# 0xPolygonZero/plonky

Hardware: AMD Instinct MI355X
Metric: MSM Mpairs/sec + NTT Melems/sec, 2^20 Tweedledee, 1/2/4/8 GPU (higher is better)
Workload: dtype u32; 1 GPU; 2^20 TweedledeeBase forward NTT + 2^20-pair tweedledee MSM per GPU per step; log_n=20, curve=tweedledee

## Files before the change

### plonky_amd/csrc/msm_geom.h

```cpp
#pragma once
#include <stddef.h>
#include <stdint.h>
#include <stdio.h>

#include "../../include/plonky_hip.h"
#include "glv_params.cuh"

namespace plk {

constexpr int ACC_THREADS = 128;

constexpr int MSM_MAX_PLANE_PARTS = 16;
constexpr int MSM_TF_MAX_WINDOW = 16;
constexpr int MSM_MAX_WINDOW = 21;
constexpr uint32_t CODE_INVALID = 0xFFFFFFFFu;
constexpr int ORD_THREADS = 256;
constexpr int ORD_TILE = 4096;
constexpr int ORD_MAX_BINS = 1024;
constexpr int ORD_MAX_FINE = 11;
constexpr int ORD_BIN_THREADS = 512;
constexpr uint32_t ORD_SEG = 8192;
constexpr int ORD_SEG_EPT = (int)(ORD_SEG / ORD_BIN_THREADS);
static_assert(3 * (4u << ORD_MAX_FINE) + 4 * ORD_BIN_THREADS + 6 * ORD_SEG <= 160 * 1024, "k_ord_bin_scatter's LDS tile must fit a gfx950 CU");
constexpr uint32_t ORD2_BIN_CAP = 32768;
constexpr int PLANE_THREADS = 512;
constexpr int FINAL_FUSE_WINDOWS = 4;
constexpr int FINAL_THREADS = 512;
constexpr int COMBINE_THREADS = 512;
constexpr uint32_t HEAD_NONE = 0xFFFFFFFFu;
constexpr uint32_t HEAVY_HEADS = 32;
constexpr uint32_t HEAVY_CHUNK = 2048;

struct OrdCfg {
    int c;
    int windows;
    uint32_t window_buckets;
    int fine_bits;
    int nbins;
    uint32_t spt;
    uint32_t sub;
    uint32_t nt1;
    int raw_signed;
    uint32_t entries_cap;
    uint32_t ent_stride;
    uint32_t ent_first;
    int perm;
    uint32_t bin_lo, bin_hi;
};

struct TailGeom {
    uint32_t buckets, heavy_cap, tail_wbuckets;
    int lpb_log;
    int two_level;
    int L, H, g_log, lpl_log;
    int table_free, windows;
    int tail_windows;
    int plane_blocks;
    int planes;
    int tail_shift;
    int transposed;
    int many_heads;
};

constexpr int META_BIN_TOTAL = 0;
constexpr int META_BIN_BASE = META_BIN_TOTAL + ORD_MAX_BINS;
constexpr int META_SEG_BASE = META_BIN_BASE + ORD_MAX_BINS + 1;
constexpr int META_DONE = META_SEG_BASE + ORD_MAX_BINS + 1;
constexpr int META_FINAL_DONE = META_DONE + 1;
constexpr int META_DYN_CHUNK = META_DONE + 2;
constexpr int META_LIVE_COUNT = META_DONE + 3;
constexpr int META_WORDS = META_DONE + 8;

enum MsmPart {
    PART_TMP,
    PART_SORTED,
    PART_CNT1,
    PART_CNT2,
    PART_META,
    PART_OFF,
    PART_P_START,
    PART_P_HEAD,
    PART_HEAD_LIVE,
    PART_BUCKET,
    PART_HEAVY,
    PART_HEAVY_PART,
    PART_LINE_PART,
    PART_PLANE_PART,
    PART_WIN_PTS,
    MSM_WORK_PARTS
};

inline size_t head_lanes_padded(size_t max_lanes) { return (max_lanes + ACC_THREADS + 15) & ~(size_t)15; }

struct MsmKnob {
    bool set = false;
    int v = 0;
};
struct MsmKnobs {
    MsmKnob window;
    MsmKnob window_2p14;
    MsmKnob window_tf;
    MsmKnob glog;
    int slice = 0;
    int comb = -1;
    bool no_glv = false;
    bool order_v1 = false;
};

struct MsmGeom {
    int c = 0;
    int windows = 0;
    uint32_t buckets = 0;
    uint32_t wbuckets = 0;
    bool table_free = false;
    bool glv = false;
    size_t n_eff = 0;
    OrdCfg ord{};
    TailGeom tail{};
    uint32_t chunk = 24;
    size_t max_lanes = 0;
    uint32_t heavy_cap = 0;
    size_t part_bytes[MSM_WORK_PARTS] = {};
    char error[192] = {};
};

constexpr int msm_scalar_bits(int curve) {
    return curve == PLK_CURVE_BLS12_377 ? 253 : (curve >= PLK_CURVE_TWEEDLEDEE && curve <= PLK_CURVE_VESTA) ? 255 : -1;
}

inline int ilog2_ceil(uint64_t v) {
    int b = 0;
    while (((uint64_t)1 << b) < v) ++b;
    return b;
}

inline int choose_window(size_t n, int curve, const MsmKnobs& knobs) {
    int lg = 0;
    while (((size_t)1 << (lg + 1)) <= n) ++lg;
    const int bits = msm_scalar_bits(curve) + 1;
    auto digits = [&](int c) { return (bits + c - 1) / c; };
    auto top_bits = [&](int c) { return bits - (digits(c) - 1) * c; };
    int c;
    if (lg >= 14) {
        double best = 0;
        c = 0;
        for (int t = 10; t <= MSM_MAX_WINDOW - 1; ++t) {
            const double acc = 10.0 * (double)n * digits(t);
            const double cost = acc + 28.0 * (double)((size_t)1 << (t - 1)) + (2 * top_bits(t) < t ? 0.1 * acc : 0.0);
            if (c == 0 || cost < best) {
                best = cost;
                c = t;
            }
        }
// ... 176 lines not shown
```

### plonky_amd/csrc/msm_order.hip

```cpp
#include "msm_dev.cuh"
#include "glv.cuh"
#include <cstdlib>

namespace plk {


struct OrdRaw {
    uint4 lo, hi;
};
PLK_DI OrdRaw ord_load_scalar(const uint4* __restrict__ scalars, size_t i, bool live) {
    OrdRaw r;
    r.lo = r.hi = make_uint4(0u, 0u, 0u, 0u);
    if (live) {
        r.lo = scalars[i * 2];
        r.hi = scalars[i * 2 + 1];
    }
    return r;
}
template <class SP> PLK_DI void ord_park_loaded(const OrdRaw& r, uint32_t* s_lim, int tid, bool raw_signed) {
    static_assert(SP::NL == 8, "scalar fields are 256-bit");
    Fe<SP> s;
    s.v[0] = r.lo.x; s.v[1] = r.lo.y; s.v[2] = r.lo.z; s.v[3] = r.lo.w;
    s.v[4] = r.hi.x; s.v[5] = r.hi.y; s.v[6] = r.hi.z; s.v[7] = r.hi.w;
    if (!raw_signed) s = fe_to_canonical<SP>(s);
#pragma unroll
    for (int k = 0; k < 8; ++k) s_lim[k * ORD_THREADS + tid] = s.v[k];
}
template <class SP> PLK_DI void ord_park_scalar(const uint4* __restrict__ scalars, size_t i, uint32_t* s_lim, int tid, bool raw_signed) {
    ord_park_loaded<SP>(ord_load_scalar(scalars, i, true), s_lim, tid, raw_signed);
}
PLK_DI uint32_t ord_digit(const uint32_t* s_lim, int tid, int j, const OrdCfg& cfg, uint32_t& carry) {
    const int c = cfg.c;
    const uint32_t mask = (1u << c) - 1u, half = 1u << (c - 1);
    const int bp = j * c, li = bp >> 5, sh = bp & 31;
    uint64_t two = li < 8 ? s_lim[li * ORD_THREADS + tid] : 0u;
    if (li + 1 < 8) two |= (uint64_t)s_lim[(li + 1) * ORD_THREADS + tid] << 32;
    const uint32_t v = ((uint32_t)(two >> sh) & mask) + carry;
    const uint32_t neg = v > half ? 1u : 0u;
    const uint32_t mag = neg ? (1u << c) - v : v;
    carry = neg;
    if (mag == 0) return CODE_INVALID;
    const uint32_t flip = cfg.raw_signed ? s_lim[7 * ORD_THREADS + tid] >> 31 : 0u;
    return ((mag - 1u + (uint32_t)j * cfg.window_buckets) << 1) | (neg ^ flip);
}

PLK_DI bool ord_bin_kept(uint32_t bin, const OrdCfg& cfg) { return bin - cfg.bin_lo < cfg.bin_hi - cfg.bin_lo; }

PLK_DI uint32_t block_excl_prefix(uint32_t v, uint32_t* s_tmp, uint32_t* total = nullptr) {
    const int t = threadIdx.x, lane = t & 63, wave = t >> 6, nw = blockDim.x >> 6;
    uint32_t inc = v;
#pragma unroll
    for (int d = 1; d < 64; d <<= 1) {
        const uint32_t u = __shfl_up(inc, d);
        if (lane >= d) inc += u;
    }
    if (lane == 63) s_tmp[wave] = inc;
    __syncthreads();
    uint32_t base = 0, all = 0;
    for (int w = 0; w < nw; ++w) {
        const uint32_t x = s_tmp[w];
        if (w < wave) base += x;
        all += x;
    }
    if (total) *total = all;
    __syncthreads();
    return base + inc - v;
}
PLK_DI void block_excl_scan4(uint32_t* s_data, int count, uint32_t* s_tmp) {
    const int t = threadIdx.x;
    uint32_t v[4], sum = 0;
#pragma unroll
    for (int k = 0; k < 4; ++k) {
        const int idx = t * 4 + k;
        v[k] = idx < count ? s_data[idx] : 0u;
        sum += v[k];
    }
    uint32_t run = block_excl_prefix(sum, s_tmp);
#pragma unroll
    for (int k = 0; k < 4; ++k) {
        const int idx = t * 4 + k;
        if (idx < count) s_data[idx] = run;
        run += v[k];
    }
    __syncthreads();
// ... 220 lines not shown
    __syncthreads();
#pragma unroll
    for (int k = 0; k < ORD_SEG_EPT; ++k)
        if (lo + tid + k * ORD_BIN_THREADS < hi) atomicAdd(&s_hist[(code[k] >> 1) & fmask], 1u);
    __syncthreads();
    for (int k = tid; k < nf; k += ORD_BIN_THREADS) cnt2[((size_t)blockIdx.x << fine_bits) + k] = s_hist[k];
}
__global__ void __launch_bounds__(ORD_BIN_THREADS) k_ord_bin_scatter(const uint2* __restrict__ tmp, const uint32_t* __restrict__ bin_base,
                                                                     const uint32_t* __restrict__ seg_base, int fine_bits, int nbins, uint32_t buckets,
                                                                     const uint32_t* __restrict__ cnt2, uint32_t* __restrict__ off,
                                                                     uint32_t* __restrict__ sorted, uint32_t entries_cap) {
    __shared__ uint32_t s_glob[1 << ORD_MAX_FINE], s_loc[1 << ORD_MAX_FINE], s_cur[1 << ORD_MAX_FINE];
    __shared__ uint32_t s_tmp[ORD_BIN_THREADS];
    __shared__ uint32_t s_out[ORD_SEG];
    __shared__ uint16_t s_fine[ORD_SEG];
    const int tid = threadIdx.x;
    uint32_t bin, seg, lo, hi;
    if (!ord_segment(seg_base, bin_base, nbins, blockIdx.x, bin, seg, lo, hi)) {
        const uint32_t extra = blockIdx.x - seg_base[nbins];
        if (extra < (uint32_t)nbins && bin_base[extra + 1] == bin_base[extra]) {
            const int nf = 1 << fine_bits;
            for (int k = tid; k < nf; k += ORD_BIN_THREADS) off[((size_t)extra << fine_bits) + k] = bin_base[extra];
        }
        if (extra == 0 && tid == 0) off[buckets] = bin_base[nbins];
        return;
    }
    const int nf = 1 << fine_bits;
    const uint32_t fmask = (uint32_t)nf - 1u;
    uint2 ent[ORD_SEG_EPT];
#pragma unroll
    for (int k = 0; k < ORD_SEG_EPT; ++k) {
        const uint32_t p = lo + tid + k * ORD_BIN_THREADS;
        ent[k] = tmp[p < hi ? p : lo];
    }
    const uint32_t s0 = seg_base[bin], s1 = seg_base[bin + 1];
    for (int k = tid; k < nf; k += ORD_BIN_THREADS) {
        uint32_t tot = 0, before = 0, own = 0;
        for (uint32_t sg = s0; sg < s1; ++sg) {
            const uint32_t v = cnt2[((size_t)sg << fine_bits) + k];
            if (sg - s0 < seg) before += v;
            if (sg - s0 == seg) own = v;
            tot += v;
        }
        s_glob[k] = tot;
        s_cur[k] = before;
        s_loc[k] = own;
    }
    __syncthreads();
    block_excl_scan4(s_glob, nf, s_tmp);
    block_excl_scan4(s_loc, nf, s_tmp);
    const uint32_t bb = bin_base[bin];
    for (int k = tid; k < nf; k += ORD_BIN_THREADS) {
        const uint32_t o = bb + s_glob[k];
        if (seg == 0) off[((size_t)bin << fine_bits) + k] = o;
        s_glob[k] = o + s_cur[k];
        s_cur[k] = s_loc[k];
    }
    __syncthreads();
#pragma unroll
    for (int k = 0; k < ORD_SEG_EPT; ++k) {
        if (lo + tid + k * ORD_BIN_THREADS >= hi) continue;
        const uint2 e = ent[k];
        const uint32_t f = (e.x >> 1) & fmask;
        const uint32_t idx = atomicAdd(&s_cur[f], 1u);
        if (PLK_CHK(idx < ORD_SEG, CHK_SEG_STAGE)) {
            s_out[idx] = (e.y << 1) | (e.x & 1u);
            s_fine[idx] = (uint16_t)f;
        }
    }
    __syncthreads();
    const uint32_t count = hi - lo;
    for (uint32_t i = tid; i < count; i += ORD_BIN_THREADS) {
        const uint32_t f = s_fine[i];
        const uint32_t at = s_glob[f] + (i - s_loc[f]);
        if (PLK_CHK(at < entries_cap, CHK_SORTED_INDEX)) sorted[at] = s_out[i];
    }
}


constexpr int ORD2_TS = 1024;
constexpr int ORD2_THREADS = 512;
constexpr int ORD2_SPT = ORD2_TS / ORD2_THREADS;
constexpr int ORD2_MAX_WINDOWS = 16;
constexpr uint32_t ORD2_MAX_TILES = 8192;
PLK_DI uint32_t ord2_record(uint32_t sign, uint32_t fine, int j, uint32_t loc) { return sign | (fine << 1) | ((uint32_t)j << 12) | (loc << 16); }
PLK_DI uint32_t ord_digit_at(const uint32_t* s_lim, int stride, int slot, int j, const OrdCfg& cfg, uint32_t& carry) {
    const int c = cfg.c;
    const uint32_t mask = (1u << c) - 1u, half = 1u << (c - 1);
    const int bp = j * c, li = bp >> 5, sh = bp & 31;
    uint64_t two = li < 8 ? s_lim[li * stride + slot] : 0u;
    if (li + 1 < 8) two |= (uint64_t)s_lim[(li + 1) * stride + slot] << 32;
    const uint32_t v = ((uint32_t)(two >> sh) & mask) + carry;
    const uint32_t neg = v > half ? 1u : 0u;
    const uint32_t mag = neg ? (1u << c) - v : v;
    carry = neg;
    if (mag == 0) return CODE_INVALID;
    const uint32_t flip = cfg.raw_signed ? s_lim[7 * stride + slot] >> 31 : 0u;
    return ((mag - 1u + (uint32_t)j * cfg.window_buckets) << 1) | (neg ^ flip);
}
struct OrdWalk {
    uint32_t w[8];
    uint32_t carry, flip;
};
template <class SP> PLK_DI void ord_walk_start(OrdWalk& s, const Fe<SP>& canon, const OrdCfg& cfg) {
#pragma unroll
    for (int k = 0; k < 8; ++k) s.w[k] = canon.v[k];
    s.carry = 0;
    s.flip = cfg.raw_signed ? canon.v[7] >> 31 : 0u;
}
PLK_DI uint32_t ord_walk_next(OrdWalk& s, int j, const OrdCfg& cfg) {
    const int c = cfg.c;
    const uint32_t mask = (1u << c) - 1u, half = 1u << (c - 1);
    const uint32_t v = (s.w[0] & mask) + s.carry;
#pragma unroll
    for (int k = 0; k < 7; ++k) s.w[k] = (s.w[k] >> c) | (s.w[k + 1] << (32 - c));
    s.w[7] >>= c;
    const uint32_t neg = v > half ? 1u : 0u;
    const uint32_t mag = neg ? (1u << c) - v : v;
    s.carry = neg;
    if (mag == 0) return CODE_INVALID;
    return ((mag - 1u + (uint32_t)j * cfg.window_buckets) << 1) | (neg ^ s.flip);
}
template <class C>
__global__ void __launch_bounds__(ORD2_THREADS) k_ord_tiles(const uint4* __restrict__ scalars, size_t n, OrdCfg cfg, uint32_t* __restrict__ cnt1,
                                                            uint32_t* __restrict__ bin_total, uint32_t* __restrict__ tmp) {
    using SP = typename C::SP;
    static_assert(SP::NL == 8, "scalar fields are 256-bit");
    __shared__ uint32_t s_cnt[ORD_MAX_BINS], s_base[ORD_MAX_BINS];
    __shared__ uint32_t s_tmp[ORD2_THREADS];
    __shared__ uint32_t s_total;
    extern __shared__ __attribute__((aligned(16))) uint32_t s_ent[];
    const int tid = threadIdx.x;
    const uint32_t tile = blockIdx.x;
    const uint32_t cap = (uint32_t)ORD2_TS * (uint32_t)cfg.windows;
    static_assert(ORD2_SPT == 2, "two scalars per thread, held in named registers (an indexed array of them is promoted to LDS by the compiler: 32 KiB)");
    const size_t i0 = (size_t)tile * ORD2_TS + tid, i1 = i0 + ORD2_THREADS;
    const bool live0 = i0 < n, live1 = i1 < n;
    const OrdRaw raw0 = ord_load_scalar(scalars, i0, live0), raw1 = ord_load_scalar(scalars, i1, live1);
    for (int k = tid; k < cfg.nbins; k += ORD2_THREADS) s_cnt[k] = 0;
    auto canonical = [&](const OrdRaw& r) {
        Fe<SP> sc;
        sc.v[0] = r.lo.x; sc.v[1] = r.lo.y; sc.v[2] = r.lo.z; sc.v[3] = r.lo.w;
        sc.v[4] = r.hi.x; sc.v[5] = r.hi.y; sc.v[6] = r.hi.z; sc.v[7] = r.hi.w;
        if (!cfg.raw_signed) sc = fe_to_canonical<SP>(sc);
        return sc;
    };
    const Fe<SP> canon0 = canonical(raw0), canon1 = canonical(raw1);
    __syncthreads();
    const int cbits = cfg.c - 1 - cfg.fine_bits;
    const uint32_t bmask = (1u << cbits) - 1u;
    uint32_t code0[ORD2_MAX_WINDOWS], code1[ORD2_MAX_WINDOWS];
    {
        OrdWalk w0, w1;
        ord_walk_start<SP>(w0, canon0, cfg);
        ord_walk_start<SP>(w1, canon1, cfg);
#pragma unroll
        for (int j = 0; j < ORD2_MAX_WINDOWS; ++j) {
            code0[j] = (j < cfg.windows && live0) ? ord_walk_next(w0, j, cfg) : CODE_INVALID;
            code1[j] = (j < cfg.windows && live1) ? ord_walk_next(w1, j, cfg) : CODE_INVALID;
            if (code0[j] != CODE_INVALID && !ord_bin_kept((code0[j] >> 1) & bmask, cfg)) code0[j] = CODE_INVALID;
            if (code1[j] != CODE_INVALID && !ord_bin_kept((code1[j] >> 1) & bmask, cfg)) code1[j] = CODE_INVALID;
        }
    }
#pragma unroll
    for (int j = 0; j < ORD2_MAX_WINDOWS; ++j) {
        if (code0[j] != CODE_INVALID) atomicAdd(&s_cnt[(code0[j] >> 1) & bmask], 1u);
        if (code1[j] != CODE_INVALID) atomicAdd(&s_cnt[(code1[j] >> 1) & bmask], 1u);
    }
    __syncthreads();
    for (int k = tid; k < cfg.nbins; k += ORD2_THREADS) s_base[k] = s_cnt[k];
    __syncthreads();
    block_excl_scan4(s_base, cfg.nbins, s_tmp);
    if (tid == 0) s_total = s_base[cfg.nbins - 1] + s_cnt[cfg.nbins - 1];
    for (int k = tid; k < cfg.nbins; k += ORD2_THREADS) {
        const uint32_t cn = s_cnt[k];
        cnt1[(size_t)k * cfg.nt1 + tile] = (s_base[k] << 16) | cn;
        if (cn) atomicAdd(&bin_total[k], cn);
    }
    __syncthreads();
#pragma unroll
    for (int j = 0; j < ORD2_MAX_WINDOWS; ++j) {
        if (code0[j] != CODE_INVALID) {
            const uint32_t slot = atomicAdd(&s_base[(code0[j] >> 1) & bmask], 1u);
            if (PLK_CHK(slot < cap, CHK_TILE_STAGE)) s_ent[slot] = ord2_record(code0[j] & 1u, code0[j] >> (cbits + 1), j, (uint32_t)tid);
        }
        if (code1[j] != CODE_INVALID) {
            const uint32_t slot = atomicAdd(&s_base[(code1[j] >> 1) & bmask], 1u);
            if (PLK_CHK(slot < cap, CHK_TILE_STAGE)) s_ent[slot] = ord2_record(code1[j] & 1u, code1[j] >> (cbits + 1), j, (uint32_t)(ORD2_THREADS + tid));
        }
    }
    __syncthreads();
    const uint32_t total = s_total;
    uint32_t* __restrict__ region = tmp + (size_t)tile * cap;
    for (uint32_t i = tid; i < total; i += ORD2_THREADS)
        if (PLK_CHK((size_t)tile * cap + i < (size_t)cfg.nt1 * cap, CHK_TMP_INDEX)) region[i] = s_ent[i];
}

__global__ void __launch_bounds__(256) k_ord_scan_bins(uint32_t* __restrict__ bin_total, int nbins, uint32_t* __restrict__ bin_base,
                                                       uint32_t* __restrict__ seg_base, uint32_t* __restrict__ dyn_chunk, uint32_t chunk_cfg,
                                                       uint32_t lanes_cfg, uint32_t hot) {
    __shared__ uint32_t s_sum[256];
    __shared__ uint32_t s_bins[ORD_MAX_BINS], s_tot[ORD_MAX_BINS];
    for (int k = threadIdx.x; k < nbins; k += 256) {
        s_tot[k] = s_bins[k] = bin_total[k];
        bin_total[k] = 0;
    }
    __syncthreads();
    const uint32_t last_total = s_bins[nbins - 1];
    block_excl_scan4(s_bins, nbins, s_sum);
    for (int k = threadIdx.x; k < nbins; k += 256) bin_base[k] = s_bins[k];
    if (threadIdx.x == 0) {
        const uint32_t total = s_bins[nbins - 1] + last_total;
        bin_base[nbins] = total;
        uint32_t ch = lanes_cfg ? (total + lanes_cfg - 1) / lanes_cfg : chunk_cfg;
        if (ch < 8u) ch = 8u;
        if (ch > chunk_cfg) ch = chunk_cfg;
        dyn_chunk[0] = ch;
    }
    __syncthreads();
    for (int k = threadIdx.x; k < nbins; k += 256) s_bins[k] = s_tot[k] > hot ? (s_tot[k] + ORD_SEG - 1) / ORD_SEG : 0u;
    __syncthreads();
    const uint32_t last_segs = s_bins[nbins - 1];
    block_excl_scan4(s_bins, nbins, s_sum);
    for (int k = threadIdx.x; k < nbins; k += 256) seg_base[k] = s_bins[k];
    if (threadIdx.x == 0) seg_base[nbins] = s_bins[nbins - 1] + last_segs;
}

struct Ord2Seg {
    uint32_t bin, seg, plo, phi;
};
PLK_DI bool ord2_segment(const uint32_t* __restrict__ seg_base, const uint32_t* __restrict__ bin_base, int nbins, uint32_t blk, Ord2Seg& sg) {
    if (blk >= seg_base[nbins]) return false;
    uint32_t a = 0, b = (uint32_t)nbins;
    while (b - a > 1) {
        const uint32_t m = (a + b) >> 1;
        if (seg_base[m] <= blk) a = m; else b = m;
    }
    sg.bin = a;
    sg.seg = blk - seg_base[a];
    sg.plo = sg.seg * ORD_SEG;
    sg.phi = min(bin_base[a + 1] - bin_base[a], sg.plo + ORD_SEG);
    return true;
}
PLK_DI void ord2_prefix(const uint32_t* __restrict__ cnt1, uint32_t nt, uint32_t bin, uint32_t* s_run, uint32_t* s_pre, uint32_t* s_tmp) {
    const int tid = threadIdx.x, nthr = blockDim.x;
    const uint32_t per = (nt + nthr - 1) / nthr;
    const uint32_t lo = min(nt, (uint32_t)tid * per), hi = min(nt, lo + per);
    uint32_t sum = 0;
    for (uint32_t t = lo; t < hi; ++t) {
        const uint32_t w = cnt1[(size_t)bin * nt + t];
        s_run[t] = w;
        sum += w & 0xFFFFu;
    }
    uint32_t total = 0;
    uint32_t run = block_excl_prefix(sum, s_tmp, &total);
    for (uint32_t t = lo; t < hi; ++t) {
        s_pre[t] = run;
        run += s_run[t] & 0xFFFFu;
    }
    if (tid == 0) {
        s_pre[nt] = total;
        s_run[nt] = 0;
    }
    __syncthreads();
}
template <int THREADS = ORD_BIN_THREADS, int EPT = ORD_SEG_EPT>
PLK_DI void ord2_gather(const uint32_t* __restrict__ tmp, const uint32_t* s_run, const uint32_t* s_pre, uint32_t nt, uint32_t cap, uint32_t plo, uint32_t phi,
                        uint32_t (&rec)[EPT], uint32_t (&til)[EPT]) {
    uint32_t t[EPT];
#pragma unroll
    for (int k = 0; k < EPT; ++k) t[k] = 0;
    uint32_t top = 1;
    while (top * 2 <= nt) top *= 2;
    for (uint32_t step = top; step; step >>= 1) {
#pragma unroll
        for (int k = 0; k < EPT; ++k) {
            const uint32_t p = plo + threadIdx.x + (uint32_t)k * THREADS;
            const uint32_t cand = t[k] + step;
            if (cand < nt && s_pre[cand] <= p) t[k] = cand;
        }
    }
#pragma unroll
    for (int k = 0; k < EPT; ++k) {
        const uint32_t p = plo + threadIdx.x + (uint32_t)k * THREADS;
        til[k] = t[k];
        rec[k] = 0;
        if (p < phi) rec[k] = tmp[(size_t)t[k] * cap + (s_run[t[k]] >> 16) + (p - s_pre[t[k]])];
    }
}
__global__ void __launch_bounds__(ORD_BIN_THREADS) k_ord_bin_count2(const uint32_t* __restrict__ tmp, const uint32_t* __restrict__ cnt1, uint32_t nt, uint32_t cap,
                                                                    const uint32_t* __restrict__ bin_base, const uint32_t* __restrict__ seg_base, int fine_bits,
                                                                    int nbins, uint32_t* __restrict__ cnt2) {
    __shared__ uint32_t s_hist[1 << ORD_MAX_FINE];
    __shared__ uint32_t s_tmp[ORD_BIN_THREADS];
    extern __shared__ __attribute__((aligned(16))) uint32_t s_dyn[];
    uint32_t* s_run = s_dyn;
    uint32_t* s_pre = s_dyn + (nt + 1);
    const int tid = threadIdx.x;
    const int nf = 1 << fine_bits;
    const uint32_t fmask = (uint32_t)nf - 1u;
    for (uint32_t blk = blockIdx.x;; blk += gridDim.x) {
        Ord2Seg sg;
        if (!ord2_segment(seg_base, bin_base, nbins, blk, sg)) return;
        for (int k = tid; k < nf; k += ORD_BIN_THREADS) s_hist[k] = 0;
        ord2_prefix(cnt1, nt, sg.bin, s_run, s_pre, s_tmp);
        uint32_t rec[ORD_SEG_EPT], til[ORD_SEG_EPT];
        ord2_gather(tmp, s_run, s_pre, nt, cap, sg.plo, sg.phi, rec, til);
#pragma unroll
        for (int k = 0; k < ORD_SEG_EPT; ++k)
            if (sg.plo + tid + k * ORD_BIN_THREADS < sg.phi) atomicAdd(&s_hist[(rec[k] >> 1) & fmask], 1u);
        __syncthreads();
        for (int k = tid; k < nf; k += ORD_BIN_THREADS) cnt2[((size_t)blk << fine_bits) + k] = s_hist[k];
        __syncthreads();
    }
}
__global__ void __launch_bounds__(ORD_BIN_THREADS) k_ord_bin_scatter2(const uint32_t* __restrict__ tmp, const uint32_t* __restrict__ cnt1, uint32_t nt, uint32_t cap,
                                                                      const uint32_t* __restrict__ bin_base, const uint32_t* __restrict__ seg_base, int fine_bits,
                                                                      int nbins, uint32_t buckets, const uint32_t* __restrict__ cnt2, uint32_t* __restrict__ off,
                                                                      uint32_t* __restrict__ sorted, uint32_t entries_cap, uint32_t ent_stride, uint32_t ent_first) {
    __shared__ uint32_t s_tmp[ORD_BIN_THREADS];
    __shared__ uint32_t s_out[ORD_SEG];
    __shared__ uint16_t s_fine[ORD_SEG];
    extern __shared__ __attribute__((aligned(16))) uint32_t s_dyn[];
    uint32_t* s_glob = s_dyn;
    uint32_t* s_loc = s_dyn + ((size_t)1 << fine_bits);
    uint32_t* s_cur = s_dyn + ((size_t)2 << fine_bits);
    uint32_t* s_run = s_dyn + ((size_t)3 << fine_bits);
    uint32_t* s_pre = s_run + (nt + 1);
    const int tid = threadIdx.x;
    for (uint32_t blk = blockIdx.x;; blk += gridDim.x) {
    Ord2Seg sg;
    if (!ord2_segment(seg_base, bin_base, nbins, blk, sg)) return;
    const int nf = 1 << fine_bits;
    const uint32_t fmask = (uint32_t)nf - 1u;
    const uint32_t bin = sg.bin, seg = sg.seg;
    ord2_prefix(cnt1, nt, bin, s_run, s_pre, s_tmp);
    uint32_t rec[ORD_SEG_EPT], til[ORD_SEG_EPT];
    ord2_gather(tmp, s_run, s_pre, nt, cap, sg.plo, sg.phi, rec, til);
    const uint32_t s0 = seg_base[bin], s1 = seg_base[bin + 1];
    for (int k = tid; k < nf; k += ORD_BIN_THREADS) {
        uint32_t tot = 0, before = 0, own = 0;
        for (uint32_t sgi = s0; sgi < s1; ++sgi) {
            const uint32_t v = cnt2[((size_t)sgi << fine_bits) + k];
            if (sgi - s0 < seg) before += v;
            if (sgi - s0 == seg) own = v;
            tot += v;
        }
        s_glob[k] = tot;
        s_cur[k] = before;
        s_loc[k] = own;
    }
    __syncthreads();
    block_excl_scan4(s_glob, nf, s_tmp);
    block_excl_scan4(s_loc, nf, s_tmp);
    const uint32_t bb = bin_base[bin];
    for (int k = tid; k < nf; k += ORD_BIN_THREADS) {
        const uint32_t o = bb + s_glob[k];
        if (seg == 0) off[((size_t)bin << fine_bits) + k] = o;
        s_glob[k] = o + s_cur[k];
        s_cur[k] = s_loc[k];
    }
    __syncthreads();
#pragma unroll
    for (int k = 0; k < ORD_SEG_EPT; ++k) {
        if (sg.plo + tid + k * ORD_BIN_THREADS >= sg.phi) continue;
        const uint32_t r = rec[k];
        const uint32_t f = (r >> 1) & fmask;
        const uint32_t idx = atomicAdd(&s_cur[f], 1u);
        if (PLK_CHK(idx < ORD_SEG, CHK_SEG_STAGE)) {
            const uint32_t entry = ((r >> 12) & 15u) * ent_stride + ent_first + til[k] * (uint32_t)ORD2_TS + (r >> 16);
            s_out[idx] = (entry << 1) | (r & 1u);
            s_fine[idx] = (uint16_t)f;
        }
    }
    __syncthreads();
    const uint32_t count = sg.phi - sg.plo;
    for (uint32_t i = tid; i < count; i += ORD_BIN_THREADS) {
        const uint32_t f = s_fine[i];
        const uint32_t at = s_glob[f] + (i - s_loc[f]);
        if (PLK_CHK(at < entries_cap, CHK_SORTED_INDEX)) sorted[at] = s_out[i];
    }
    __syncthreads();
    }
}

constexpr int ORD2_SORT_THREADS = 1024;
constexpr int ORD2_SORT_UNROLL = 8;
template <class F>
PLK_DI void ord2_for_runs(const uint32_t* __restrict__ tmp, const uint32_t* s_run, uint32_t nt, uint32_t cap, F&& f) {
    const uint32_t hw = threadIdx.x >> 5, hl = threadIdx.x & 31u;
    constexpr uint32_t HW = ORD2_SORT_THREADS / 32;
    for (uint32_t t0 = hw; t0 < nt; t0 += HW * ORD2_SORT_UNROLL) {
        uint32_t w[ORD2_SORT_UNROLL], r[ORD2_SORT_UNROLL];
#pragma unroll
        for (int u = 0; u < ORD2_SORT_UNROLL; ++u) {
            const uint32_t t = t0 + (uint32_t)u * HW;
            w[u] = t < nt ? s_run[t] : 0u;
            r[u] = 0;
            if (hl < (w[u] & 0xFFFFu)) r[u] = tmp[(size_t)t * cap + (w[u] >> 16) + hl];
        }
#pragma unroll
        for (int u = 0; u < ORD2_SORT_UNROLL; ++u) {
            const uint32_t t = t0 + (uint32_t)u * HW, cnt = w[u] & 0xFFFFu;
            if (hl < cnt) f(r[u], t);
            for (uint32_t i = hl + 32u; i < cnt; i += 32u) f(tmp[(size_t)t * cap + (w[u] >> 16) + i], t);
        }
    }
}
template <bool CACHE>
__global__ void __launch_bounds__(ORD2_SORT_THREADS) k_ord_bin_sort(const uint32_t* __restrict__ tmp, const uint32_t* __restrict__ cnt1, uint32_t nt, uint32_t cap,
                                                                    const uint32_t* __restrict__ bin_base, int fine_bits, int nbins, uint32_t buckets,
                                                                    uint32_t* __restrict__ off, uint32_t* __restrict__ sorted, uint32_t entries_cap,
                                                                    uint32_t ent_stride, uint32_t ent_first) {
    __shared__ uint32_t s_tmp[ORD2_SORT_THREADS];
    extern __shared__ __attribute__((aligned(16))) uint32_t s_dyn[];
    const int nf = 1 << fine_bits;
    uint32_t* s_out = s_dyn;
    uint32_t* s_cur = s_dyn + ORD2_BIN_CAP;
    uint32_t* s_run = s_cur + nf;
    const int tid = threadIdx.x;
    const uint32_t bin = blockIdx.x;
    const uint32_t bb = bin_base[bin], total = bin_base[bin + 1] - bb;
    if (bin == 0 && tid == 0) off[buckets] = bin_base[nbins];
    if (total == 0) {
        for (int k = tid; k < nf; k += ORD2_SORT_THREADS) off[((size_t)bin << fine_bits) + k] = bb;
        return;
    }
    if (total > ORD2_BIN_CAP) return;
    const uint32_t fmask = (uint32_t)nf - 1u;
    for (int k = tid; k < nf; k += ORD2_SORT_THREADS) s_cur[k] = 0;
    for (uint32_t t = tid; t < nt; t += ORD2_SORT_THREADS) s_run[t] = cnt1[(size_t)bin * nt + t];
    __syncthreads();
    auto count = [&](uint32_t r, uint32_t) { atomicAdd(&s_cur[(r >> 1) & fmask], 1u); };
    auto place = [&](uint32_t r, uint32_t t) {
        const uint32_t idx = atomicAdd(&s_cur[(r >> 1) & fmask], 1u);
        const uint32_t entry = ((r >> 12) & 15u) * ent_stride + ent_first + t * (uint32_t)ORD2_TS + (r >> 16);
        if (PLK_CHK(idx < ORD2_BIN_CAP, CHK_SEG_STAGE)) s_out[idx] = (entry << 1) | (r & 1u);
    };
    constexpr int STEPS = 4;
    constexpr uint32_t HW = ORD2_SORT_THREADS / 32;
    const uint32_t hw = (uint32_t)tid >> 5, hl = (uint32_t)tid & 31u;
    uint32_t rc[STEPS * ORD2_SORT_UNROLL];
    if constexpr (CACHE) {
#pragma unroll
        for (int st = 0; st < STEPS; ++st) {
#pragma unroll
            for (int u = 0; u < ORD2_SORT_UNROLL; ++u) {
                const uint32_t t = hw + (uint32_t)(st * ORD2_SORT_UNROLL + u) * HW;
                const uint32_t w = t < nt ? s_run[t] : 0u;
                rc[st * ORD2_SORT_UNROLL + u] = 0;
                if (hl < (w & 0xFFFFu)) rc[st * ORD2_SORT_UNROLL + u] = tmp[(size_t)t * cap + (w >> 16) + hl];
            }
#pragma unroll
            for (int u = 0; u < ORD2_SORT_UNROLL; ++u) {
                const uint32_t t = hw + (uint32_t)(st * ORD2_SORT_UNROLL + u) * HW;
                const uint32_t w = t < nt ? s_run[t] : 0u, cnt = w & 0xFFFFu;
                if (hl < cnt) count(rc[st * ORD2_SORT_UNROLL + u], t);
                for (uint32_t i = hl + 32u; i < cnt; i += 32u) count(tmp[(size_t)t * cap + (w >> 16) + i], t);
            }
        }
    } else {
        ord2_for_runs(tmp, s_run, nt, cap, count);
    }
    __syncthreads();
    block_excl_scan4(s_cur, nf, s_tmp);
    for (int k = tid; k < nf; k += ORD2_SORT_THREADS) off[((size_t)bin << fine_bits) + k] = bb + s_cur[k];
    __syncthreads();
    if constexpr (CACHE) {
#pragma unroll
        for (int st = 0; st < STEPS; ++st)
#pragma unroll
            for (int u = 0; u < ORD2_SORT_UNROLL; ++u) {
                const uint32_t t = hw + (uint32_t)(st * ORD2_SORT_UNROLL + u) * HW;
                const uint32_t w = t < nt ? s_run[t] : 0u, cnt = w & 0xFFFFu;
                if (hl < cnt) place(rc[st * ORD2_SORT_UNROLL + u], t);
                for (uint32_t i = hl + 32u; i < cnt; i += 32u) place(tmp[(size_t)t * cap + (w >> 16) + i], t);
            }
    } else {
        ord2_for_runs(tmp, s_run, nt, cap, place);
    }
    __syncthreads();
    for (uint32_t i = tid; i < total; i += ORD2_SORT_THREADS)
        if (PLK_CHK(bb + i < entries_cap, CHK_SORTED_INDEX)) sorted[bb + i] = s_out[i];
}

template <class C> int msm_launch_glv_split(const void* d_scalars, size_t n, void* halves, hipStream_t stream) {
    k_glv_split<C><<<(unsigned)((n + 255) / 256), 256, 0, stream>>>((const uint4*)d_scalars, n, (uint4*)halves);
    PLK_HIP_TRY(hipGetLastError());
    return PLK_OK;
}
static bool order_tiles2(const OrdCfg& o) { return o.perm != 0; }
template <class C> int msm_launch_order_stage(int stage, const OrdCfg& o, const OrdBuffers& b, hipStream_t stream) {
    const bool one_level = o.fine_bits == 0;
    uint32_t *const bin_total = b.meta + META_BIN_TOTAL, *const bin_base = b.meta + META_BIN_BASE, *const seg_base = b.meta + META_SEG_BASE;
    if (order_tiles2(o)) {
        const uint32_t cap = (uint32_t)ORD2_TS * (uint32_t)o.windows;
        if (stage == 0) {
            const size_t lds = (size_t)cap * 4;
            (void)hipFuncSetAttribute((const void*)k_ord_tiles<C>, hipFuncAttributeMaxDynamicSharedMemorySize, ORD2_TS * ORD2_MAX_WINDOWS * 4);
            k_ord_tiles<C><<<o.nt1, ORD2_THREADS, lds, stream>>>((const uint4*)b.scalars, b.n, o, (uint32_t*)b.cnt1, bin_total, (uint32_t*)b.tmp);
            k_ord_scan_bins<<<1, 256, 0, stream>>>(bin_total, o.nbins, bin_base, seg_base, b.meta + META_DYN_CHUNK, b.chunk, b.lanes, ORD2_BIN_CAP);
        } else if (stage == 2) {
            const size_t entries = b.n * (size_t)o.windows;
            const size_t hot_bins = entries / ORD2_BIN_CAP < (size_t)o.nbins ? entries / ORD2_BIN_CAP : (size_t)o.nbins;
            const unsigned segs = (unsigned)(entries / ORD_SEG + hot_bins + 1);
            const size_t lds = (size_t)2 * (o.nt1 + 1) * 4, lds_s = lds + ((size_t)3 << o.fine_bits) * 4;
            const size_t lds_b = ((size_t)ORD2_BIN_CAP + ((size_t)1 << o.fine_bits) + o.nt1) * 4;
            static const bool no_cache = getenv("PLK_MSM_BINSORT_NOCACHE") != nullptr;
            if (o.nt1 <= 1024u && !no_cache) {
                (void)hipFuncSetAttribute((const void*)k_ord_bin_sort<true>, hipFuncAttributeMaxDynamicSharedMemorySize, (int)lds_b);
                k_ord_bin_sort<true><<<o.nbins, ORD2_SORT_THREADS, lds_b, stream>>>((const uint32_t*)b.tmp, (const uint32_t*)b.cnt1, o.nt1, cap, bin_base, o.fine_bits,
                                                                                   o.nbins, b.buckets, (uint32_t*)b.off, (uint32_t*)b.sorted, o.entries_cap, o.ent_stride,
                                                                                   o.ent_first);
            } else {
                (void)hipFuncSetAttribute((const void*)k_ord_bin_sort<false>, hipFuncAttributeMaxDynamicSharedMemorySize, (int)lds_b);
                k_ord_bin_sort<false><<<o.nbins, ORD2_SORT_THREADS, lds_b, stream>>>((const uint32_t*)b.tmp, (const uint32_t*)b.cnt1, o.nt1, cap, bin_base, o.fine_bits,
                                                                                    o.nbins, b.buckets, (uint32_t*)b.off, (uint32_t*)b.sorted, o.entries_cap, o.ent_stride,
                                                                                    o.ent_first);
            }
            const unsigned hot_grid = segs < 512u ? segs : 512u;
            k_ord_bin_count2<<<hot_grid, ORD_BIN_THREADS, lds, stream>>>((const uint32_t*)b.tmp, (const uint32_t*)b.cnt1, o.nt1, cap, bin_base, seg_base, o.fine_bits,
                                                                   o.nbins, (uint32_t*)b.cnt2);
            k_ord_bin_scatter2<<<hot_grid, ORD_BIN_THREADS, lds_s, stream>>>((const uint32_t*)b.tmp, (const uint32_t*)b.cnt1, o.nt1, cap, bin_base, seg_base,
                                                                               o.fine_bits, o.nbins, b.buckets, (const uint32_t*)b.cnt2, (uint32_t*)b.off,
                                                                               (uint32_t*)b.sorted, o.entries_cap, o.ent_stride, o.ent_first);
        }
        PLK_HIP_TRY(hipGetLastError());
        return PLK_OK;
    }
    if (stage == 0) {
        k_ord_count<C><<<o.nt1, ORD_THREADS, 0, stream>>>((const uint4*)b.scalars, b.n, o, (uint32_t*)b.cnt1);
        k_ord_scan1<<<o.nbins, 256, 0, stream>>>((uint32_t*)b.cnt1, o.nt1, o.nbins, bin_total, bin_base, seg_base, b.meta + META_DONE, b.meta + META_DYN_CHUNK,
                                                 b.chunk, b.lanes, one_level ? (uint32_t*)b.off : nullptr);
    } else if (stage == 1) {
        k_ord_scatter<C><<<o.nt1, ORD_THREADS, 0, stream>>>((const uint4*)b.scalars, b.n, o, (const uint32_t*)b.cnt1, bin_base, (uint2*)b.tmp,
                                                            one_level ? (uint32_t*)b.sorted : nullptr);
    } else if (!one_level) {
        const unsigned segs = (unsigned)(b.n * (size_t)o.windows / ORD_SEG + o.nbins + 1);
        k_ord_bin_count<<<segs, ORD_BIN_THREADS, 0, stream>>>((const uint2*)b.tmp, bin_base, seg_base, o.fine_bits, o.nbins, (uint32_t*)b.cnt2);
        k_ord_bin_scatter<<<segs + o.nbins, ORD_BIN_THREADS, 0, stream>>>((const uint2*)b.tmp, bin_base, seg_base, o.fine_bits, o.nbins, b.buckets,
                                                                          (const uint32_t*)b.cnt2, (uint32_t*)b.off, (uint32_t*)b.sorted, o.entries_cap);
    }
    PLK_HIP_TRY(hipGetLastError());
    return PLK_OK;
}
template <class C> int msm_launch_digits(const void* d_scalars, size_t n, const OrdCfg& o, void* d_digits, hipStream_t stream) {
    k_ord_digits<C><<<(unsigned)((n + ORD_THREADS - 1) / ORD_THREADS), ORD_THREADS, 0, stream>>>((const uint4*)d_scalars, n, o, (int32_t*)d_digits);
    PLK_HIP_TRY(hipGetLastError());
    return PLK_OK;
}
#define PLK_ORD_INSTANTIATE(C)                                                                     \
    template int msm_launch_glv_split<C>(const void*, size_t, void*, hipStream_t);                \
    template int msm_launch_order_stage<C>(int, const OrdCfg&, const OrdBuffers&, hipStream_t);   \
    template int msm_launch_digits<C>(const void*, size_t, const OrdCfg&, void*, hipStream_t);
PLK_FOR_EACH_CURVE(PLK_ORD_INSTANTIATE)
#undef PLK_ORD_INSTANTIATE

PLK_CHK_READER(msm_order_checked_failures)

}
```

Baseline: 1507 M units/s (1 unit = 1 NTT element or 1 MSM scalar-point pair; components below).

## Fold bin scan and hot-bin path into the bin-sort kernel

Removes the single-block bin-scan kernel and the two hot-bin segment kernels (count2/scatter2) from the tiled ordering path. Each bin-sort block now computes its own prefix over the bin totals, sets the dynamic chunk, and resets the totals through a last-block atomic counter. Oversized bins scatter directly to global memory with atomics instead of going through the segmented path. It also caches the hipFuncSetAttribute calls per device and caps tiles at 2048. This cuts three launches per MSM, at the cost of a redundant per-block scan and slower uncoalesced writes for hot bins.

Result: no change. 1516 M units/s (1 unit = 1 NTT element or 1 MSM scalar-point pair; components below) (median of 3 runs) (+0.6%).

```diff
diff --git a/plonky_amd/csrc/msm_geom.h b/plonky_amd/csrc/msm_geom.h
--- a/plonky_amd/csrc/msm_geom.h
+++ b/plonky_amd/csrc/msm_geom.h
@@ -69,6 +69,7 @@
 constexpr int META_FINAL_DONE = META_DONE + 1;
 constexpr int META_DYN_CHUNK = META_DONE + 2;
 constexpr int META_LIVE_COUNT = META_DONE + 3;
+constexpr int META_SORT_DONE = META_DONE + 4;
 constexpr int META_WORDS = META_DONE + 8;
 
 enum MsmPart {
diff --git a/plonky_amd/csrc/msm_order.hip b/plonky_amd/csrc/msm_order.hip
--- a/plonky_amd/csrc/msm_order.hip
+++ b/plonky_amd/csrc/msm_order.hip
@@ -1,5 +1,6 @@
 #include "msm_dev.cuh"
 #include "glv.cuh"
+#include <atomic>
 #include <cstdlib>
 
 namespace plk {
@@ -386,7 +387,7 @@
 constexpr int ORD2_THREADS = 512;
 constexpr int ORD2_SPT = ORD2_TS / ORD2_THREADS;
 constexpr int ORD2_MAX_WINDOWS = 16;
-constexpr uint32_t ORD2_MAX_TILES = 8192;
+constexpr uint32_t ORD2_MAX_TILES = 2048;
 PLK_DI uint32_t ord2_record(uint32_t sign, uint32_t fine, int j, uint32_t loc) { return sign | (fine << 1) | ((uint32_t)j << 12) | (loc << 16); }
 PLK_DI uint32_t ord_digit_at(const uint32_t* s_lim, int stride, int slot, int j, const OrdCfg& cfg, uint32_t& carry) {
     const int c = cfg.c;
@@ -500,194 +501,6 @@
         if (PLK_CHK((size_t)tile * cap + i < (size_t)cfg.nt1 * cap, CHK_TMP_INDEX)) region[i] = s_ent[i];
 }
 
-__global__ void __launch_bounds__(256) k_ord_scan_bins(uint32_t* __restrict__ bin_total, int nbins, uint32_t* __restrict__ bin_base,
-                                                       uint32_t* __restrict__ seg_base, uint32_t* __restrict__ dyn_chunk, uint32_t chunk_cfg,
-                                                       uint32_t lanes_cfg, uint32_t hot) {
-    __shared__ uint32_t s_sum[256];
-    __shared__ uint32_t s_bins[ORD_MAX_BINS], s_tot[ORD_MAX_BINS];
-    for (int k = threadIdx.x; k < nbins; k += 256) {
-        s_tot[k] = s_bins[k] = bin_total[k];
-        bin_total[k] = 0;
-    }
-    __syncthreads();
-    const uint32_t last_total = s_bins[nbins - 1];
-    block_excl_scan4(s_bins, nbins, s_sum);
-    for (int k = threadIdx.x; k < nbins; k += 256) bin_base[k] = s_bins[k];
-    if (threadIdx.x == 0) {
-        const uint32_t total = s_bins[nbins - 1] + last_total;
-        bin_base[nbins] = total;
-        uint32_t ch = lanes_cfg ? (total + lanes_cfg - 1) / lanes_cfg : chunk_cfg;
-        if (ch < 8u) ch = 8u;
-        if (ch > chunk_cfg) ch = chunk_cfg;
-        dyn_chunk[0] = ch;
-    }
-    __syncthreads();
-    for (int k = threadIdx.x; k < nbins; k += 256) s_bins[k] = s_tot[k] > hot ? (s_tot[k] + ORD_SEG - 1) / ORD_SEG : 0u;
-    __syncthreads();
-    const uint32_t last_segs = s_bins[nbins - 1];
-    block_excl_scan4(s_bins, nbins, s_sum);
-    for (int k = threadIdx.x; k < nbins; k += 256) seg_base[k] = s_bins[k];
-    if (threadIdx.x == 0) seg_base[nbins] = s_bins[nbins - 1] + last_segs;
-}
-
-struct Ord2Seg {
-    uint32_t bin, seg, plo, phi;
-};
-PLK_DI bool ord2_segment(const uint32_t* __restrict__ seg_base, const uint32_t* __restrict__ bin_base, int nbins, uint32_t blk, Ord2Seg& sg) {
-    if (blk >= seg_base[nbins]) return false;
-    uint32_t a = 0, b = (uint32_t)nbins;
-    while (b - a > 1) {
-        const uint32_t m = (a + b) >> 1;
-        if (seg_base[m] <= blk) a = m; else b = m;
-    }
-    sg.bin = a;
-    sg.seg = blk - seg_base[a];
-    sg.plo = sg.seg * ORD_SEG;
-    sg.phi = min(bin_base[a + 1] - bin_base[a], sg.plo + ORD_SEG);
-    return true;
-}
-PLK_DI void ord2_prefix(const uint32_t* __restrict__ cnt1, uint32_t nt, uint32_t bin, uint32_t* s_run, uint32_t* s_pre, uint32_t* s_tmp) {
-    const int tid = threadIdx.x, nthr = blockDim.x;
-    const uint32_t per = (nt + nthr - 1) / nthr;
-    const uint32_t lo = min(nt, (uint32_t)tid * per), hi = min(nt, lo + per);
-    uint32_t sum = 0;
-    for (uint32_t t = lo; t < hi; ++t) {
-        const uint32_t w = cnt1[(size_t)bin * nt + t];
-        s_run[t] = w;
-        sum += w & 0xFFFFu;
-    }
-    uint32_t total = 0;
-    uint32_t run = block_excl_prefix(sum, s_tmp, &total);
-    for (uint32_t t = lo; t < hi; ++t) {
-        s_pre[t] = run;
-        run += s_run[t] & 0xFFFFu;
-    }
-    if (tid == 0) {
-        s_pre[nt] = total;
-        s_run[nt] = 0;
-    }
-    __syncthreads();
-}
-template <int THREADS = ORD_BIN_THREADS, int EPT = ORD_SEG_EPT>
-PLK_DI void ord2_gather(const uint32_t* __restrict__ tmp, const uint32_t* s_run, const uint32_t* s_pre, uint32_t nt, uint32_t cap, uint32_t plo, uint32_t phi,
-                        uint32_t (&rec)[EPT], uint32_t (&til)[EPT]) {
-    uint32_t t[EPT];
-#pragma unroll
-    for (int k = 0; k < EPT; ++k) t[k] = 0;
-    uint32_t top = 1;
-    while (top * 2 <= nt) top *= 2;
-    for (uint32_t step = top; step; step >>= 1) {
-#pragma unroll
-        for (int k = 0; k < EPT; ++k) {
-            const uint32_t p = plo + threadIdx.x + (uint32_t)k * THREADS;
-            const uint32_t cand = t[k] + step;
-            if (cand < nt && s_pre[cand] <= p) t[k] = cand;
-        }
-    }
-#pragma unroll
-    for (int k = 0; k < EPT; ++k) {
-        const uint32_t p = plo + threadIdx.x + (uint32_t)k * THREADS;
-        til[k] = t[k];
-        rec[k] = 0;
-        if (p < phi) rec[k] = tmp[(size_t)t[k] * cap + (s_run[t[k]] >> 16) + (p - s_pre[t[k]])];
-    }
-}
-__global__ void __launch_bounds__(ORD_BIN_THREADS) k_ord_bin_count2(const uint32_t* __restrict__ tmp, const uint32_t* __restrict__ cnt1, uint32_t nt, uint32_t cap,
-                                                                    const uint32_t* __restrict__ bin_base, const uint32_t* __restrict__ seg_base, int fine_bits,
-                                                                    int nbins, uint32_t* __restrict__ cnt2) {
-    __shared__ uint32_t s_hist[1 << ORD_MAX_FINE];
-    __shared__ uint32_t s_tmp[ORD_BIN_THREADS];
-    extern __shared__ __attribute__((aligned(16))) uint32_t s_dyn[];
-    uint32_t* s_run = s_dyn;
-    uint32_t* s_pre = s_dyn + (nt + 1);
-    const int tid = threadIdx.x;
-    const int nf = 1 << fine_bits;
-    const uint32_t fmask = (uint32_t)nf - 1u;
-    for (uint32_t blk = blockIdx.x;; blk += gridDim.x) {
-        Ord2Seg sg;
-        if (!ord2_segment(seg_base, bin_base, nbins, blk, sg)) return;
-        for (int k = tid; k < nf; k += ORD_BIN_THREADS) s_hist[k] = 0;
-        ord2_prefix(cnt1, nt, sg.bin, s_run, s_pre, s_tmp);
-        uint32_t rec[ORD_SEG_EPT], til[ORD_SEG_EPT];
-        ord2_gather(tmp, s_run, s_pre, nt, cap, sg.plo, sg.phi, rec, til);
-#pragma unroll
-        for (int k = 0; k < ORD_SEG_EPT; ++k)
-            if (sg.plo + tid + k * ORD_BIN_THREADS < sg.phi) atomicAdd(&s_hist[(rec[k] >> 1) & fmask], 1u);
-        __syncthreads();
-        for (int k = tid; k < nf; k += ORD_BIN_THREADS) cnt2[((size_t)blk << fine_bits) + k] = s_hist[k];
-        __syncthreads();
-    }
-}
-__global__ void __launch_bounds__(ORD_BIN_THREADS) k_ord_bin_scatter2(const uint32_t* __restrict__ tmp, const uint32_t* __restrict__ cnt1, uint32_t nt, uint32_t cap,
-                                                                      const uint32_t* __restrict__ bin_base, const uint32_t* __restrict__ seg_base, int fine_bits,
-                                                                      int nbins, uint32_t buckets, const uint32_t* __restrict__ cnt2, uint32_t* __restrict__ off,
-                                                                      uint32_t* __restrict__ sorted, uint32_t entries_cap, uint32_t ent_stride, uint32_t ent_first) {
-    __shared__ uint32_t s_tmp[ORD_BIN_THREADS];
-    __shared__ uint32_t s_out[ORD_SEG];
-    __shared__ uint16_t s_fine[ORD_SEG];
-    extern __shared__ __attribute__((aligned(16))) uint32_t s_dyn[];
-    uint32_t* s_glob = s_dyn;
-    uint32_t* s_loc = s_dyn + ((size_t)1 << fine_bits);
-    uint32_t* s_cur = s_dyn + ((size_t)2 << fine_bits);
-    uint32_t* s_run = s_dyn + ((size_t)3 << fine_bits);
-    uint32_t* s_pre = s_run + (nt + 1);
-    const int tid = threadIdx.x;
-    for (uint32_t blk = blockIdx.x;; blk += gridDim.x) {
-    Ord2Seg sg;
-    if (!ord2_segment(seg_base, bin_base, nbins, blk, sg)) return;
-    const int nf = 1 << fine_bits;
-    const uint32_t fmask = (uint32_t)nf - 1u;
-    const uint32_t bin = sg.bin, seg = sg.seg;
-    ord2_prefix(cnt1, nt, bin, s_run, s_pre, s_tmp);
-    uint32_t rec[ORD_SEG_EPT], til[ORD_SEG_EPT];
-    ord2_gather(tmp, s_run, s_pre, nt, cap, sg.plo, sg.phi, rec, til);
-    const uint32_t s0 = seg_base[bin], s1 = seg_base[bin + 1];
-    for (int k = tid; k < nf; k += ORD_BIN_THREADS) {
-        uint32_t tot = 0, before = 0, own = 0;
-        for (uint32_t sgi = s0; sgi < s1; ++sgi) {
-            const uint32_t v = cnt2[((size_t)sgi << fine_bits) + k];
-            if (sgi - s0 < seg) before += v;
-            if (sgi - s0 == seg) own = v;
-            tot += v;
-        }
-        s_glob[k] = tot;
-        s_cur[k] = before;
-        s_loc[k] = own;
-    }
-    __syncthreads();
-    block_excl_scan4(s_glob, nf, s_tmp);
-    block_excl_scan4(s_loc, nf, s_tmp);
-    const uint32_t bb = bin_base[bin];
-    for (int k = tid; k < nf; k += ORD_BIN_THREADS) {
-        const uint32_t o = bb + s_glob[k];
-        if (seg == 0) off[((size_t)bin << fine_bits) + k] = o;
-        s_glob[k] = o + s_cur[k];
-        s_cur[k] = s_loc[k];
-    }
-    __syncthreads();
-#pragma unroll
-    for (int k = 0; k < ORD_SEG_EPT; ++k) {
-        if (sg.plo + tid + k * ORD_BIN_THREADS >= sg.phi) continue;
-        const uint32_t r = rec[k];
-        const uint32_t f = (r >> 1) & fmask;
-        const uint32_t idx = atomicAdd(&s_cur[f], 1u);
-        if (PLK_CHK(idx < ORD_SEG, CHK_SEG_STAGE)) {
-            const uint32_t entry = ((r >> 12) & 15u) * ent_stride + ent_first + til[k] * (uint32_t)ORD2_TS + (r >> 16);
-            s_out[idx] = (entry << 1) | (r & 1u);
-            s_fine[idx] = (uint16_t)f;
-        }
-    }
-    __syncthreads();
-    const uint32_t count = sg.phi - sg.plo;
-    for (uint32_t i = tid; i < count; i += ORD_BIN_THREADS) {
-        const uint32_t f = s_fine[i];
-        const uint32_t at = s_glob[f] + (i - s_loc[f]);
-        if (PLK_CHK(at < entries_cap, CHK_SORTED_INDEX)) sorted[at] = s_out[i];
-    }
-    __syncthreads();
-    }
-}
-
 constexpr int ORD2_SORT_THREADS = 1024;
 constexpr int ORD2_SORT_UNROLL = 8;
 template <class F>
@@ -713,10 +526,13 @@
 }
 template <bool CACHE>
 __global__ void __launch_bounds__(ORD2_SORT_THREADS) k_ord_bin_sort(const uint32_t* __restrict__ tmp, const uint32_t* __restrict__ cnt1, uint32_t nt, uint32_t cap,
-                                                                    const uint32_t* __restrict__ bin_base, int fine_bits, int nbins, uint32_t buckets,
+                                                                    uint32_t* bin_total, uint32_t* __restrict__ sort_done, uint32_t* __restrict__ dyn_chunk,
+                                                                    uint32_t chunk_cfg, uint32_t lanes_cfg, int fine_bits, int nbins, uint32_t buckets,
                                                                     uint32_t* __restrict__ off, uint32_t* __restrict__ sorted, uint32_t entries_cap,
                                                                     uint32_t ent_stride, uint32_t ent_first) {
+    static_assert(ORD_MAX_BINS <= ORD2_SORT_THREADS, "one thread per bin in the prefix over the bins' totals");
     __shared__ uint32_t s_tmp[ORD2_SORT_THREADS];
+    __shared__ uint32_t s_bin[2];
     extern __shared__ __attribute__((aligned(16))) uint32_t s_dyn[];
     const int nf = 1 << fine_bits;
     uint32_t* s_out = s_dyn;
@@ -724,22 +540,48 @@
     uint32_t* s_run = s_cur + nf;
     const int tid = threadIdx.x;
     const uint32_t bin = blockIdx.x;
-    const uint32_t bb = bin_base[bin], total = bin_base[bin + 1] - bb;
-    if (bin == 0 && tid == 0) off[buckets] = bin_base[nbins];
+    const uint32_t mine = tid < nbins ? bin_total[tid] : 0u;
+    for (int k = tid; k < nf; k += ORD2_SORT_THREADS) s_cur[k] = 0;
+    for (uint32_t t = tid; t < nt; t += ORD2_SORT_THREADS) s_run[t] = cnt1[(size_t)bin * nt + t];
+    uint32_t entries = 0;
+    const uint32_t before = block_excl_prefix(mine, s_tmp, &entries);
+    if ((uint32_t)tid == bin) {
+        s_bin[0] = before;
+        s_bin[1] = mine;
+    }
+    if (tid < 64) {
+        uint32_t seen = 0;
+        if (tid == 0) seen = atomicAdd(sort_done, 1u);
+        seen = __shfl(seen, 0);
+        if (seen == gridDim.x - 1u) {
+            for (int k = tid; k < nbins; k += 64) bin_total[k] = 0;
+            if (tid == 0) *sort_done = 0;
+        }
+    }
+    __syncthreads();
+    const uint32_t bb = s_bin[0], total = s_bin[1];
+    if (bin == 0 && tid == 0) {
+        off[buckets] = entries;
+        uint32_t ch = lanes_cfg ? (entries + lanes_cfg - 1) / lanes_cfg : chunk_cfg;
+        if (ch < 8u) ch = 8u;
+        if (ch > chunk_cfg) ch = chunk_cfg;
+        dyn_chunk[0] = ch;
+    }
     if (total == 0) {
         for (int k = tid; k < nf; k += ORD2_SORT_THREADS) off[((size_t)bin << fine_bits) + k] = bb;
         return;
     }
-    if (total > ORD2_BIN_CAP) return;
+    const bool hot = total > ORD2_BIN_CAP;
     const uint32_t fmask = (uint32_t)nf - 1u;
-    for (int k = tid; k < nf; k += ORD2_SORT_THREADS) s_cur[k] = 0;
-    for (uint32_t t = tid; t < nt; t += ORD2_SORT_THREADS) s_run[t] = cnt1[(size_t)bin * nt + t];
-    __syncthreads();
     auto count = [&](uint32_t r, uint32_t) { atomicAdd(&s_cur[(r >> 1) & fmask], 1u); };
     auto place = [&](uint32_t r, uint32_t t) {
         const uint32_t idx = atomicAdd(&s_cur[(r >> 1) & fmask], 1u);
         const uint32_t entry = ((r >> 12) & 15u) * ent_stride + ent_first + t * (uint32_t)ORD2_TS + (r >> 16);
-        if (PLK_CHK(idx < ORD2_BIN_CAP, CHK_SEG_STAGE)) s_out[idx] = (entry << 1) | (r & 1u);
+        if (hot) {
+            if (PLK_CHK(bb + idx < entries_cap, CHK_SORTED_INDEX)) sorted[bb + idx] = (entry << 1) | (r & 1u);
+        } else if (PLK_CHK(idx < ORD2_BIN_CAP, CHK_SEG_STAGE)) {
+            s_out[idx] = (entry << 1) | (r & 1u);
+        }
     };
     constexpr int STEPS = 4;
     constexpr uint32_t HW = ORD2_SORT_THREADS / 32;
@@ -783,6 +625,7 @@
     } else {
         ord2_for_runs(tmp, s_run, nt, cap, place);
     }
+    if (hot) return;
     __syncthreads();
     for (uint32_t i = tid; i < total; i += ORD2_SORT_THREADS)
         if (PLK_CHK(bb + i < entries_cap, CHK_SORTED_INDEX)) sorted[bb + i] = s_out[i];
@@ -794,6 +637,17 @@
     return PLK_OK;
 }
 static bool order_tiles2(const OrdCfg& o) { return o.perm != 0; }
+static int ord_allow_lds(const void* kernel, size_t bytes, std::atomic<uint32_t>& done) {
+    int dev = 0;
+    PLK_HIP_TRY(hipGetDevice(&dev));
+    const uint32_t bit = dev >= 0 && dev < 32 ? 1u << dev : 0u;
+    if (bit && (done.load(std::memory_order_acquire) & bit)) return PLK_OK;
+    PLK_HIP_TRY(hipFuncSetAttribute(kernel, hipFuncAttributeMaxDynamicSharedMemorySize, (int)bytes));
+    done.fetch_or(bit, std::memory_order_release);
+    return PLK_OK;
+}
+constexpr size_t ORD2_SORT_LDS_MAX = ((size_t)ORD2_BIN_CAP + ((size_t)1 << ORD_MAX_FINE) + ORD2_MAX_TILES) * 4;
+static_assert(ORD2_SORT_LDS_MAX + ORD2_SORT_THREADS * 4 + 8 <= 160 * 1024, "k_ord_bin_sort's LDS must fit a gfx950 CU");
 template <class C> int msm_launch_order_stage(int stage, const OrdCfg& o, const OrdBuffers& b, hipStream_t stream) {
     const bool one_level = o.fine_bits == 0;
     uint32_t *const bin_total = b.meta + META_BIN_TOTAL, *const bin_base = b.meta + META_BIN_BASE, *const seg_base = b.meta + META_SEG_BASE;
@@ -801,33 +655,27 @@
         const uint32_t cap = (uint32_t)ORD2_TS * (uint32_t)o.windows;
         if (stage == 0) {
             const size_t lds = (size_t)cap * 4;
-            (void)hipFuncSetAttribute((const void*)k_ord_tiles<C>, hipFuncAttributeMaxDynamicSharedMemorySize, ORD2_TS * ORD2_MAX_WINDOWS * 4);
+            static std::atomic<uint32_t> allowed{0};
+            PLK_TRY(ord_allow_lds((const void*)k_ord_tiles<C>, (size_t)ORD2_TS * ORD2_MAX_WINDOWS * 4, allowed));
             k_ord_tiles<C><<<o.nt1, ORD2_THREADS, lds, stream>>>((const uint4*)b.scalars, b.n, o, (uint32_t*)b.cnt1, bin_total, (uint32_t*)b.tmp);
-            k_ord_scan_bins<<<1, 256, 0, stream>>>(bin_total, o.nbins, bin_base, seg_base, b.meta + META_DYN_CHUNK, b.chunk, b.lanes, ORD2_BIN_CAP);
         } else if (stage == 2) {
-            const size_t entries = b.n * (size_t)o.windows;
-            const size_t hot_bins = entries / ORD2_BIN_CAP < (size_t)o.nbins ? entries / ORD2_BIN_CAP : (size_t)o.nbins;
-            const unsigned segs = (unsigned)(entries / ORD_SEG + hot_bins + 1);
-            const size_t lds = (size_t)2 * (o.nt1 + 1) * 4, lds_s = lds + ((size_t)3 << o.fine_bits) * 4;
             const size_t lds_b = ((size_t)ORD2_BIN_CAP + ((size_t)1 << o.fine_bits) + o.nt1) * 4;
+            if (lds_b > ORD2_SORT_LDS_MAX) return set_error(PLK_ERR_INVALID_ARG, "bucket ordering: %u tiles of %d fine bits exceed k_ord_bin_sort's LDS", o.nt1, o.fine_bits);
             static const bool no_cache = getenv("PLK_MSM_BINSORT_NOCACHE") != nullptr;
+            static std::atomic<uint32_t> allowed_cache{0}, allowed_plain{0};
             if (o.nt1 <= 1024u && !no_cache) {
-                (void)hipFuncSetAttribute((const void*)k_ord_bin_sort<true>, hipFuncAttributeMaxDynamicSharedMemorySize, (int)lds_b);
-                k_ord_bin_sort<true><<<o.nbins, ORD2_SORT_THREADS, lds_b, stream>>>((const uint32_t*)b.tmp, (const uint32_t*)b.cnt1, o.nt1, cap, bin_base, o.fine_bits,
+                PLK_TRY(ord_allow_lds((const void*)k_ord_bin_sort<true>, ORD2_SORT_LDS_MAX, allowed_cache));
+                k_ord_bin_sort<true><<<o.nbins, ORD2_SORT_THREADS, lds_b, stream>>>((const uint32_t*)b.tmp, (const uint32_t*)b.cnt1, o.nt1, cap, bin_total,
+                                                                                   b.meta + META_SORT_DONE, b.meta + META_DYN_CHUNK, b.chunk, b.lanes, o.fine_bits,
                                                                                    o.nbins, b.buckets, (uint32_t*)b.off, (uint32_t*)b.sorted, o.entries_cap, o.ent_stride,
                                                                                    o.ent_first);
             } else {
-                (void)hipFuncSetAttribute((const void*)k_ord_bin_sort<false>, hipFuncAttributeMaxDynamicSharedMemorySize, (int)lds_b);
-                k_ord_bin_sort<false><<<o.nbins, ORD2_SORT_THREADS, lds_b, stream>>>((const uint32_t*)b.tmp, (const uint32_t*)b.cnt1, o.nt1, cap, bin_base, o.fine_bits,
+                PLK_TRY(ord_allow_lds((const void*)k_ord_bin_sort<false>, ORD2_SORT_LDS_MAX, allowed_plain));
+                k_ord_bin_sort<false><<<o.nbins, ORD2_SORT_THREADS, lds_b, stream>>>((const uint32_t*)b.tmp, (const uint32_t*)b.cnt1, o.nt1, cap, bin_total,
+                                                                                    b.meta + META_SORT_DONE, b.meta + META_DYN_CHUNK, b.chunk, b.lanes, o.fine_bits,
                                                                                     o.nbins, b.buckets, (uint32_t*)b.off, (uint32_t*)b.sorted, o.entries_cap, o.ent_stride,
                                                                                     o.ent_first);
             }
-            const unsigned hot_grid = segs < 512u ? segs : 512u;
-            k_ord_bin_count2<<<hot_grid, ORD_BIN_THREADS, lds, stream>>>((const uint32_t*)b.tmp, (const uint32_t*)b.cnt1, o.nt1, cap, bin_base, seg_base, o.fine_bits,
-                                                                   o.nbins, (uint32_t*)b.cnt2);
-            k_ord_bin_scatter2<<<hot_grid, ORD_BIN_THREADS, lds_s, stream>>>((const uint32_t*)b.tmp, (const uint32_t*)b.cnt1, o.nt1, cap, bin_base, seg_base,
-                                                                               o.fine_bits, o.nbins, b.buckets, (const uint32_t*)b.cnt2, (uint32_t*)b.off,
-                                                                               (uint32_t*)b.sorted, o.entries_cap, o.ent_stride, o.ent_first);
         }
         PLK_HIP_TRY(hipGetLastError());
         return PLK_OK;
```
